# radoslawkrolikowski/financial-market-data-analysis

Hardware: AMD Instinct MI355X
Metric: train seq/sec + 3-class acc, biGRU on synthetic order-book (higher is better)
Workload: dtype bf16; 1 GPU; model=biGRU L2 H128 bidirectional, global_batch=8192, seq_len=120, n_features=96, parallelism=dp1, bench_config=repo

## Files before the change

### fmda_amd/models/bigru.py

```python
from typing import Optional

import numpy as np
import torch
import torch.nn as nn
import torch.nn.functional as F

from ..metrics import batch_metrics


class BiGRU(nn.Module):

    def __init__(self, hidden_size, n_features, output_size, n_layers=1,
                 clip=50, dropout=0.2, spatial_dropout=True,
                 bidirectional=True):
        super().__init__()
        self.hidden_size = hidden_size
        self.n_features = n_features
        self.output_size = output_size
        self.n_layers = n_layers
        self.clip = clip
        self.dropout_p = dropout
        self.spatial_dropout = spatial_dropout
        self.bidirectional = bidirectional
        self.n_directions = 2 if bidirectional else 1
# ... 36 lines not shown
                input_seq = input_seq.permute(0, 2, 1)
                input_seq = self.spatial_dropout1d(input_seq)
                input_seq = input_seq.permute(0, 2, 1)
        elif (self.training and input_seq.is_cuda
              and input_seq.dtype == torch.bfloat16 and self.dropout_p > 0):
            from ..ops.interface import fused_dropout
            input_seq = fused_dropout(input_seq, self.dropout_p)
        else:
            input_seq = self.dropout(input_seq)
        return input_seq

    def _features_after_dropout(self, input_seq: torch.Tensor,
                                hidden: Optional[torch.Tensor] = None
                                ) -> torch.Tensor:
        if input_seq.is_cuda:
            from ..ops.interface import (bigru_stack_raw, pooled_features,
                                         pooled_features_native)
            if pooled_features_native(input_seq, self.hidden_size):
                gru_out, h_last = bigru_stack_raw(
                    input_seq, self.gru, self.n_layers, self.bidirectional,
                    self.dropout_p, self.training, hidden)
                return pooled_features(gru_out, h_last)
            gru_out, h_n = self._gru_hip(input_seq, hidden)
        else:
            gru_out, h_n = self.gru(input_seq, hidden)
        return self._pool_concat(gru_out, h_n)

    def _pool_concat(self, gru_out: torch.Tensor,
                     h_n: torch.Tensor) -> torch.Tensor:
        batch_size = gru_out.size(0)
        input_length = gru_out.size(1)
        hidden_v = h_n.view(self.n_layers, self.n_directions, batch_size,
                            self.hidden_size)
        last_hidden = hidden_v[-1].sum(dim=0)

        if gru_out.is_cuda and self.hidden_size % 2 == 0:
            from ..ops.interface import dirsum_pool
# ... 222 lines not shown
```

### fmda_amd/ops/csrc/bindings.cpp

```cpp
#include <torch/extension.h>
#include <ATen/hip/HIPContext.h>

#include <climits>
#include <cstdint>
#include <vector>

extern "C" int fmda_gru_fwd_launch(int is_bf16, int Hp, const void* gi,
                                   const void* w, const float* bhh, void* out,
                                   float* hlast, int B, int Tseq, int n_dir,
                                   const float* h0, void* out_drop,
                                   unsigned int drop_thr, float drop_scale,
                                   unsigned long long drop_seed,
                                   long gi_pitch, hipStream_t stream);
extern "C" int fmda_gru_fwd_cs_launch(const void* gi, const void* w,
                                      const float* bhh, void* out,
                                      float* hlast, void* hpub,
                                      unsigned int* cnt, int B, int Tseq,
                                      int n_dir, void* out_drop,
                                      unsigned int drop_thr,
                                      float drop_scale,
                                      unsigned long long drop_seed,
                                      long gi_pitch, hipStream_t stream);
extern "C" int fmda_gru_bwd_cs_launch(const void* gi, const void* w,
                                      const void* wt, const float* bhh,
// ... 4 lines not shown
                                      int n_dir, unsigned int drop_thr,
                                      float drop_scale,
                                      unsigned long long drop_seed,
                                      hipStream_t stream);
extern "C" int fmda_gru_bwd_launch(int is_bf16, int Hp, const void* gi,
                                   const void* w, const void* wt,
                                   const float* bhh,
                                   const void* out, const void* dout,
                                   const float* dhT, void* dgi, void* dgh,
                                   float* dh0, float* dbhh, int B, int Tseq,
                                   int n_dir, unsigned int drop_thr,
                                   float drop_scale,
                                   unsigned long long drop_seed,
                                   const float* h0, void* dgh0,
                                   hipStream_t stream);
extern "C" int fmda_mfma_selftest_launch(const void* A, const void* Bm,
                                         float* C, hipStream_t stream);
extern "C" int fmda_pool_fwd_launch(int is_bf16, const void* out, void* maxv,
                                    void* avgv, int* amax, int B, int Tseq,
                                    int H, int n_dir, int act_io, int serial,
                                    hipStream_t stream);
extern "C" int fmda_pool_features_fwd_launch(const void* out,
                                             const float* hlast, void* feat,
                                             int* amax, int B, int Tseq,
                                             int H, int n_dir,
                                             hipStream_t stream);
extern "C" int fmda_pool_features_bwd_launch(const void* dfeat,
                                             const int* amax, void* dout,
                                             float* dhlast, int B, int Tseq,
                                             int H, int n_dir, long ld,
// ... 223 lines not shown
    TORCH_CHECK(T >= 1 && stride >= 1,
                "gru_fwd_windows: T and stride must be >= 1");
    TORCH_CHECK(R >= T, "gru_fwd_windows: table has ", R,
                " rows, fewer than the window T=", T);
    const int64_t nB = (R - T) / stride + 1;
    TORCH_CHECK(nB <= INT_MAX && T <= INT_MAX,
                "gru_fwd_windows: too many windows");
    TORCH_CHECK(reinterpret_cast<uintptr_t>(gi_rows.data_ptr()) % 16 == 0,
                "gru_fwd_windows: gi_rows must be 16-byte aligned");
    return gru_fwd_dispatch(gi_rows, w, bhh, (int)nB, (int)T, n_dir, Hp,
                            is_bf16, stride * row, c10::nullopt, 0.0, 0);
}

std::vector<torch::Tensor> gru_bwd(torch::Tensor gi, torch::Tensor w,
                                   torch::Tensor bhh, torch::Tensor out,
                                   torch::Tensor dout, torch::Tensor dhT,
                                   double drop_p, int64_t drop_seed,
                                   c10::optional<torch::Tensor> h0_opt,
                                   c10::optional<torch::Tensor> wt_opt) {
    int B, T, n_dir, Hp;
    bool is_bf16;
    check_common(gi, w, bhh, B, T, n_dir, Hp, is_bf16);
    const float* h0 = nullptr;
    torch::Tensor dgh0;
    void* dgh0_ptr = nullptr;
    if (h0_opt.has_value()) {
        auto& h = h0_opt.value();
        TORCH_CHECK(h.is_cuda() && h.is_contiguous() &&
                    h.scalar_type() == torch::kFloat32 &&
                    h.sizes() == torch::IntArrayRef({n_dir, B, Hp}),
                    "h0 must be contiguous fp32 (n_dir, B, Hp)");
        h0 = h.data_ptr<float>();
        dgh0 = torch::empty({n_dir, B, (int64_t)3 * Hp}, gi.options());
        dgh0_ptr = dgh0.data_ptr();
    }
    TORCH_CHECK(out.is_contiguous() && dout.is_contiguous() &&
                dhT.is_contiguous(), "fmda gru_bwd: tensors must be contiguous");
    TORCH_CHECK(dhT.scalar_type() == torch::kFloat32, "dhT must be fp32");
    TORCH_CHECK(is_bf16 || Hp <= 256,
                "fp32 backward unsupported for Hp > 256 (LDS budget); "
                "train in bf16 for hidden sizes above 256");
    torch::Tensor dgi, dgh;
    if (getenv("FMDA_ZERO_GRADS")) {
        dgi = torch::zeros_like(gi);
        dgh = torch::zeros_like(gi);
    } else {
        dgi = torch::empty_like(gi);
        dgh = torch::empty_like(gi);
    }
    auto dh0 = torch::empty({n_dir, B, Hp},
                            gi.options().dtype(torch::kFloat32));
    const bool column_split = is_bf16 && Hp == 512 && h0 == nullptr;
    const int64_t db_rows = fmda_gru_bwd_db_rows(is_bf16 ? 1 : 0, Hp, B,
// ... 8 lines not shown
        if (wt_opt.has_value()) {
            wt = wt_opt.value();
            TORCH_CHECK(wt.is_cuda() && wt.is_contiguous() &&
                        wt.scalar_type() == w.scalar_type() &&
                        wt.sizes() == torch::IntArrayRef(
                            {n_dir, Hp, (int64_t)3 * Hp}),
                        "wt must be contiguous (n_dir, Hp, 3Hp) in w's dtype");
        } else {
            wt = w.transpose(1, 2).contiguous();
        }
        wt_ptr = wt.data_ptr();
    }
    auto stream = at::hip::getCurrentHIPStream();
    int rc;
    const DropParams dp = drop_params(drop_p);
    if (column_split) {
        const unsigned int cs_thr = dp.thr;
        const float cs_scale = dp.scale;
        const int BR = 256;
        const int GB = (B + BR - 1) / BR;
        const int G = GB * n_dir;
        auto gpub = torch::empty({2, G, BR, (int64_t)3 * Hp}, gi.options());
        auto cnt = torch::zeros({G}, gi.options().dtype(torch::kUInt32));
        rc = fmda_gru_bwd_cs_launch(
            gi.data_ptr(), w.data_ptr(), wt_ptr, bhh.data_ptr<float>(),
            out.data_ptr(), dout.data_ptr(), dhT.data_ptr<float>(),
            dgi.data_ptr(), dgh.data_ptr(), dh0.data_ptr<float>(),
            dbpart.data_ptr<float>(), gpub.data_ptr(),
            (unsigned int*)cnt.data_ptr(), B, T, n_dir, cs_thr, cs_scale,
            (unsigned long long)drop_seed, stream.stream());
    } else {
// ... 606 lines not shown
          "table (shared rows, no materialised windows)",
          py::arg("gi_rows"), py::arg("w"), py::arg("bhh"), py::arg("T"),
          py::arg("stride") = 1);
    m.def("normalize_table", &normalize_table,
          "nan_to_num + min/max normalisation of a raw (N, F) table",
          py::arg("x"), py::arg("x_min"), py::arg("x_max"), py::arg("dtype"));
    m.def("window_batch", &window_batch,
          "gather windows of a table into a (B, T, F) batch with fused "
          "(spatial) input dropout",
          py::arg("table"), py::arg("starts"), py::arg("window"),
          py::arg("p"), py::arg("seed"), py::arg("spatial"));
    m.def("gru_bwd", &gru_bwd, "fused biGRU recurrence backward (HIP/CDNA4)",
          py::arg("gi"), py::arg("w"), py::arg("bhh"), py::arg("out"),
          py::arg("dout"), py::arg("dhT"), py::arg("drop_p") = 0.0,
          py::arg("drop_seed") = 0, py::arg("h0") = py::none(),
          py::arg("wt") = py::none());
    m.def("mfma_selftest", &mfma_selftest, "mfma fragment layout self-test");
    m.def("dropout_fused", &dropout_fused,
          "counter-based dropout (mask recomputed in backward)");
    m.def("spatial_dropout_fused", &spatial_dropout_fused,
          "channel (Dropout2d) dropout over (B, T, F) without permutes");
    m.def("ingest_row", &ingest_row,
          "streaming ingest: shift GPU window ring + normalize new row");
    m.def("pool_concat_infer", &pool_concat_infer,
          "fused [dirsum(h_last) | max | avg] concat for inference");
    m.def("head_sigmoid", &head_sigmoid,
          "linear head + sigmoid emitting probabilities");
    m.def("pool_fwd", &pool_fwd, "fused dirsum+max/avg pooling forward",
          py::arg("out"), py::arg("n_dir"), py::arg("act_dtype") = false,
          py::arg("serial") = false);
    m.def("pool_features_fwd", &pool_features_fwd,
// ... 40 lines not shown
```

### fmda_amd/ops/csrc/gru_kernels.hip

```cpp
#include <hip/hip_runtime.h>
#include <hip/hip_bf16.h>

#include "dropout_common.h"

#define FMDA_DEV __device__ __forceinline__

typedef __bf16 bf16x8_t __attribute__((ext_vector_type(8)));
typedef float f32x4_t __attribute__((ext_vector_type(4)));

namespace fmda {

#define FMDA_LOG2E 1.4426950408889634f

FMDA_DEV float fast_exp2(float x) { return __builtin_amdgcn_exp2f(x); }
FMDA_DEV float fast_rcp(float x) { return __builtin_amdgcn_rcpf(x); }

FMDA_DEV float sigmoidf(float x) {
    return fast_rcp(1.0f + fast_exp2(-x * FMDA_LOG2E));
}

FMDA_DEV float fast_tanh(float x) {
    return 1.0f - 2.0f * fast_rcp(1.0f + fast_exp2(2.0f * FMDA_LOG2E * x));
}

// ... 1074 lines not shown
                ((__bf16*)out_b)[(long)tt * out_trow + j] = hb;
            }
        }
        asm volatile("s_waitcnt lgkmcnt(0)" ::: "memory");
        __builtin_amdgcn_s_barrier();
    }

    if ((lane >> 4) == 0) {
        float* hl = hlast + (long)dir * Hp;
#pragma unroll
        for (int i = 0; i < CPW; ++i)
            hl[(wave + NW * i) * 16 + lane] = hreg[i];
    }
}

template <int BT, int Hp, int NT, int WPE, int PHASES = 7>
__global__ __attribute__((amdgpu_flat_work_group_size(NT, NT),
                          amdgpu_waves_per_eu(WPE, WPE)))
void gru_bwd_v3_kernel(const __hip_bfloat16* __restrict__ gi,
                       const __hip_bfloat16* __restrict__ w,
                       const __hip_bfloat16* __restrict__ wt,
                       const float* __restrict__ bhh,
                       const __hip_bfloat16* __restrict__ out,
                       const __hip_bfloat16* __restrict__ dout,
                       const float* __restrict__ dhT,
                       __hip_bfloat16* __restrict__ dgi,
                       __hip_bfloat16* __restrict__ dgh, float* __restrict__ dh0,
                       float* __restrict__ dbhh, int B, int Tseq, int n_dir,
                       unsigned int drop_thr, float drop_scale,
                       unsigned long long drop_seed,
                       const float* __restrict__ h0,
                       __hip_bfloat16* __restrict__ dgh0) {
    constexpr int NW = NT / 64;
    constexpr int MT = BT / 16;
    constexpr int NCT = Hp / 16;
    constexpr int CPW = NCT / NW;
    constexpr int KK = Hp / 32;
    constexpr int KK2 = (3 * Hp) / 32;
    constexpr int GP = 3 * Hp;
    constexpr int HROW = Hp * 2;
    constexpr int GP3 = 3 * Hp + 8;
    constexpr int PW = (BT * GP * 2) / 1024 / NW;
    constexpr int DOP = (BT * HROW) / 1024 / NW;
    constexpr int HBP = DOP;
    constexpr int NST = 2 * ((BT * GP * 2) / 16) / NT;
    static_assert(NCT % NW == 0 && (BT * GP * 2) % (1024 * NW) == 0 &&
                  (BT * HROW) % (1024 * NW) == 0, "tiling mismatch");
// ... 1 lines not shown
    const int tid = threadIdx.x;
    const int wave = tid >> 6;
    const int lane = tid & 63;
    const int b0 = blockIdx.x * BT;
    const int dir = blockIdx.y;
    const bool rev = (dir == 1);
    const int rows_valid = min(BT, B - b0);

    extern __shared__ __attribute__((aligned(16))) char smem[];
    char* p = smem;
    __hip_bfloat16* gi_s0 = (__hip_bfloat16*)p; p += 2 * BT * GP;
    __hip_bfloat16* gi_s1 = (__hip_bfloat16*)p; p += 2 * BT * GP;
    __hip_bfloat16* gi_s2 = (__hip_bfloat16*)p; p += 2 * BT * GP;
    __hip_bfloat16* hb_s0 = (__hip_bfloat16*)p; p += BT * HROW;
    __hip_bfloat16* hb_s1 = (__hip_bfloat16*)p; p += BT * HROW;
    __hip_bfloat16* do_s0 = (__hip_bfloat16*)p; p += BT * HROW;
    __hip_bfloat16* do_s1 = (__hip_bfloat16*)p; p += BT * HROW;
    __hip_bfloat16* dgh_s0 = (__hip_bfloat16*)p; p += 2 * BT * GP3;
    __hip_bfloat16* dgh_s1 = (__hip_bfloat16*)p; p += 2 * BT * GP3;
    float* bhh_s = (float*)p;
    auto dgh_buf = [&](int b) { return b ? dgh_s1 : dgh_s0; };
    auto gi_slot = [&](int sl) {
        return sl == 0 ? gi_s0 : (sl == 1 ? gi_s1 : gi_s2);
    };
    auto hb_buf = [&](int b) { return b ? hb_s1 : hb_s0; };
    auto do_buf = [&](int b) { return b ? do_s1 : do_s0; };

    const long gi_row = (long)Tseq * n_dir * 3 * Hp;
    const long out_row = (long)Tseq * n_dir * Hp;
    const __hip_bfloat16* gi_b = gi + (long)b0 * gi_row + (long)dir * 3 * Hp;
    __hip_bfloat16* dgi_b = dgi + (long)b0 * gi_row + (long)dir * 3 * Hp;
    __hip_bfloat16* dgh_b = dgh + (long)b0 * gi_row + (long)dir * 3 * Hp;
    const __hip_bfloat16* out_b = out + (long)b0 * out_row + (long)dir * Hp;
    const __hip_bfloat16* dout_b = dout + (long)b0 * out_row + (long)dir * Hp;

    for (int c = tid; c < 3 * Hp; c += NT)
        bhh_s[c] = bhh[(long)dir * 3 * Hp + c];

    const __hip_bfloat16* wdir = w + (long)dir * 3 * Hp * Hp;
    const __hip_bfloat16* wt_dir = wt + (long)dir * Hp * 3 * Hp;
    bf16x8_t wA[CPW][3][KK];
    bf16x8_t wB[CPW][KK2];
#pragma unroll
    for (int i = 0; i < CPW; ++i) {
        const int ct = wave + NW * i;
        const int jcol = ct * 16 + (lane & 15);
        const __bf16* wtrow = (const __bf16*)wt_dir + (long)jcol * 3 * Hp;
#pragma unroll
        for (int g = 0; g < 3; ++g)
#pragma unroll
            for (int kk = 0; kk < KK; ++kk)
                wA[i][g][kk] = load_wfragA<Hp>(wdir, Hp, ct, g, kk, lane);
#pragma unroll
// ... 3 lines not shown

    float dhreg[CPW][MT][4];
    float dbacc[CPW][4];
#pragma unroll
    for (int i = 0; i < CPW; ++i) {
#pragma unroll
        for (int g = 0; g < 4; ++g) dbacc[i][g] = 0.0f;
        const int ct = wave + NW * i;
        const int j = ct * 16 + (lane & 15);
        const float* hT = dhT + ((long)dir * B + b0) * Hp;
#pragma unroll
        for (int m = 0; m < MT; ++m)
#pragma unroll
            for (int e = 0; e < 4; ++e) {
                const int b = 16 * m + 4 * (lane >> 4) + e;
                dhreg[i][m][e] =
                    (b < rows_valid) ? hT[(long)b * Hp + j] : 0.0f;
            }
    }

    const int wavu = __builtin_amdgcn_readfirstlane(wave);
    auto glds_gi = [&](int tt, int sl) {
        const __hip_bfloat16* src_t = gi_b + (long)tt * n_dir * 3 * Hp;
        __hip_bfloat16* dst = gi_slot(sl);
#pragma unroll
        for (int k = 0; k < PW; ++k) {
            const int off = (wavu * PW + k) * 1024 + lane * 16;
            const int e = off >> 1;
            int r = e / GP;
            const int c = e % GP;
            if (r >= rows_valid) r = 0;
            glds16(src_t + (long)r * gi_row + c,
// ... 43 lines not shown
        for (int c = tid; c < BT * Hp; c += NT)
            ((__bf16*)hb_buf(buf))[c] = (__bf16)0.0f;
    };
    auto hb_read = [&](const __hip_bfloat16* hb, int b, int j) -> float {
        const int k16 = (j * 2) >> 4;
        const int ksw = k16 ^ (b & 15);
        const int within = (j * 2) & 15;
        return (float)*(const __bf16*)((const char*)hb + b * HROW +
                                       ksw * 16 + within);
    };

    {
        const int u = Tseq - 1;
        const int tt = rev ? 0 : u;
        glds_gi(tt, u % 3);
        glds_do(tt, u & 1);
        if (u > 0) {
            const int ttp = rev ? 1 : (u - 1);
            glds_hb(ttp, u & 1);
        } else {
            zero_hb(u & 1);
        }
        asm volatile("s_waitcnt vmcnt(0)" ::: "memory");
        asm volatile("s_waitcnt lgkmcnt(0)" ::: "memory");
        __builtin_amdgcn_s_barrier();
    }

    for (int u = Tseq - 1; u >= 0; --u) {
        const int q = u & 1;
        const int slot = u % 3;
        const int tt = rev ? (Tseq - 1 - u) : u;
        const bool have_next = (u > 0);
        const bool have_prev = (u + 1 < Tseq);

        if (have_next) {
            const int ttn = rev ? (Tseq - u) : (u - 1);
            glds_gi(ttn, (u - 1) % 3);
            glds_do(ttn, 1 - q);
            if (u >= 2)
                glds_hb(rev ? (Tseq + 1 - u) : (u - 2), 1 - q);
            else
                zero_hb(1 - q);
        }
        if (have_prev) {
            const int ttp = rev ? (Tseq - 2 - u) : (u + 1);
            store_tile<__hip_bfloat16, BT, NT>(
                gi_slot((u + 1) % 3), dgi_b + (long)ttp * n_dir * 3 * Hp, GP, GP,
                gi_row, rows_valid, tid);
            const int sh = rev ? (ttp + 1) : (ttp - 1);
            store_tile<__hip_bfloat16, BT, NT>(
                dgh_buf(1 - q), dgh_b + (long)sh * n_dir * 3 * Hp, GP, GP3,
                gi_row, rows_valid, tid);
        }
// ... 24 lines not shown
#pragma unroll
                    for (int m = 0; m < MT; ++m)
                        acc[i][g][m] = __builtin_amdgcn_mfma_f32_16x16x32_bf16(
                            a[m], wA[i][g][kk], acc[i][g][m], 0, 0, 0);
            }
        }
#pragma unroll
        for (int i = 0; PHASES & 2 && i < CPW; ++i) {
            const int ct = wave + NW * i;
            const int j = ct * 16 + (lane & 15);
            __bf16* grow = (__bf16*)gi_slot(slot);
            __bf16* dgrow = (__bf16*)dgh_buf(q);
            const __bf16* dorow = (const __bf16*)do_buf(q);
#pragma unroll
            for (int m = 0; m < MT; ++m) {
#pragma unroll
                for (int e = 0; e < 4; ++e) {
                    const int b = 16 * m + 4 * (lane >> 4) + e;
                    const bool live = (b < rows_valid);
                    const float gr = acc[i][0][m][e] + bhh_s[j];
                    const float gz = acc[i][1][m][e] + bhh_s[Hp + j];
                    const float hn = acc[i][2][m][e] + bhh_s[2 * Hp + j];
                    const float ir = (float)grow[b * GP + j];
                    const float iz = (float)grow[b * GP + Hp + j];
                    const float in_ = (float)grow[b * GP + 2 * Hp + j];
                    const float r = sigmoidf(ir + gr);
                    const float z = sigmoidf(iz + gz);
                    const float n = fast_tanh(in_ + r * hn);
                    const float hprev = hb_read(hbq, b, j);
                    float doval = live ? (float)dorow[b * Hp + j] : 0.0f;
                    if (drop_thr != 0u) {
                        const long o = ((long)(b0 + b) * Tseq + tt) *
                                           n_dir * Hp +
                                       (long)dir * Hp + j;
                        const unsigned long long rnd =
                            mix64(drop_seed ^ (unsigned long long)(o >> 3));
                        const unsigned int u =
                            (unsigned int)(rnd >> (8 * ((int)o & 7))) & 0xFF;
                        doval = (u < drop_thr) ? 0.0f : doval * drop_scale;
                    }
                    const float dht = dhreg[i][m][e] + doval;
                    const float dz_pre =
                        live ? dht * (hprev - n) * z * (1.0f - z) : 0.0f;
                    const float dn_pre =
                        live ? dht * (1.0f - z) * (1.0f - n * n) : 0.0f;
                    const float dr_pre =
// ... 1680 lines not shown
                               hipStream_t stream) {
    constexpr int Hp = 128;
    const size_t lds = 3 * 2 * BT * 3 * Hp + 2 * 2 * BT * Hp +
                       2 * 2 * BT * Hp + 2 * 2 * BT * (3 * Hp + 8) +
                       4 * 3 * Hp;
    auto k = gru_bwd_v3_kernel<BT, Hp, NT, 2, PHASES>;
    (void)hipFuncSetAttribute((const void*)k,
        hipFuncAttributeMaxDynamicSharedMemorySize, (int)lds);
    const dim3 grid((B + BT - 1) / BT, n_dir);
    k<<<grid, NT, lds, stream>>>(
        (const __hip_bfloat16*)gi, (const __hip_bfloat16*)w,
        (const __hip_bfloat16*)wt, bhh,
        (const __hip_bfloat16*)out, (const __hip_bfloat16*)dout, dhT,
        (__hip_bfloat16*)dgi, (__hip_bfloat16*)dgh, dh0, dbhh, B, Tseq,
        n_dir, drop_thr, drop_scale, drop_seed, h0,
        (__hip_bfloat16*)dgh0);
    return 0;
}

static bool bwd_v3_bt16() {
    static const bool small = getenv("FMDA_BWD_BT16") != nullptr;
    return small;
}

static int launch_bwd_v3_128(const void* gi, const void* w, const void* wt,
                             const float* bhh,
                             const void* out, const void* dout,
                             const float* dhT, void* dgi, void* dgh,
                             float* dh0, float* dbhh, int B, int Tseq,
                             int n_dir, unsigned int drop_thr,
                             float drop_scale, unsigned long long drop_seed,
// ... 205 lines not shown
        }
    } else {
        switch (Hp) {
            case 16: G(float, 32, 16, false, 256, false); break;
            case 32: G(float, 32, 32, false, 256, false); break;
            case 64: G(float, 32, 64, false, 256, false); break;
            case 128: G(float, 32, 128, false, 256, false); break;
            case 256: G(float, 16, 256, false, 256, false); break;
            default: return -1;
        }
    }
#undef G
    return hipGetLastError() == hipSuccess ? 0 : -4;
}

extern "C" int fmda_mfma_selftest_launch(const void* A, const void* Bm,
                                         float* C, hipStream_t stream) {
    mfma_selftest_kernel<<<1, 64, 0, stream>>>((const __hip_bfloat16*)A,
                                               (const __hip_bfloat16*)Bm, C);
    return hipGetLastError() == hipSuccess ? 0 : 1;
}

}
```

### fmda_amd/ops/interface.py

```python
import os
from typing import List, Optional, Tuple

import torch

from . import load_extension
from .blas import (chunked_colsum, chunked_outer, chunked_outer_parts,
                   enable_tunableop, split_chunks)

_ALLOWED_HP = [32, 64, 128, 256, 512]


def _pad_h(H: int) -> int:
    for hp in _ALLOWED_HP:
        if H <= hp:
            return hp
    raise ValueError(f"hidden size {H} > {_ALLOWED_HP[-1]} not supported")


def _glue_mode() -> int:
    return {"0": 0, "2": 2}.get(os.environ.get("FMDA_NATIVE_GLUE", "1"), 1)


def _native_glue() -> bool:
    return _glue_mode() >= 1
# ... 231 lines not shown
                   for g in (dmax, davg)):
                dmax, davg = dmax.contiguous(), davg.contiguous()
        else:
            dmax, davg = dmax.float().contiguous(), davg.float().contiguous()
        dout = ext.pool_bwd(dmax, davg, amax, T, n_dir, dtype)
        return dout, None


def dirsum_pool(out: torch.Tensor, n_dir: int):
    return _DirSumPool.apply(out, n_dir)


class _PooledFeatures(torch.autograd.Function):

    @staticmethod
    def forward(ctx, out, h_last):
        ext = load_extension()
        feat, amax = ext.pool_features_fwd(out.contiguous(),
                                           h_last.contiguous())
        ctx.save_for_backward(amax)
        ctx.meta = (out.shape[1], h_last.shape[0])
        return feat

    @staticmethod
    def backward(ctx, dfeat):
        ext = load_extension()
        (amax,) = ctx.saved_tensors
        T, n_dir = ctx.meta
        if (dfeat.dtype != torch.bfloat16 or dfeat.stride(1) != 1
                or dfeat.stride(0) < dfeat.shape[1]):
            dfeat = dfeat.to(torch.bfloat16).contiguous()
        d_out, d_hlast = ext.pool_features_bwd(dfeat, amax, T, n_dir)
        return d_out, d_hlast


_POOL_SMALL_GRID = 4096


def pooled_features_native(x: torch.Tensor, H: int) -> bool:
    return (_native_glue() and x.is_cuda and x.dtype == torch.bfloat16
            and H % 8 == 0 and H <= _ALLOWED_HP[-1] and _pad_h(H) == H
            and x.shape[0] * (H // 2) >= _POOL_SMALL_GRID)


def pooled_features(out: torch.Tensor, h_last: torch.Tensor) -> torch.Tensor:
    return _PooledFeatures.apply(out, h_last)


# ... 74 lines not shown
    return _HeadLoss.apply(x2d, Wc, bc, y.float(), wgt.float(), pw.float())


def _unpad_gate_rows(w, H, Hp):
    if H == Hp:
        return w
    return torch.cat([w[g * Hp:g * Hp + H] for g in range(3)], dim=0)


class _BiGRULayer(torch.autograd.Function):

    @staticmethod
    def forward(ctx, x, Hp, w_ih0, w_hh0, b_ih0, b_hh0,
                w_ih1, w_hh1, b_ih1, b_hh1, out_drop_p=0.0,
                out_drop_seed=0, h0=None):
        ext = load_extension()
        D = 2 if w_ih1 is not None else 1
        H = w_hh0.shape[1]
        dtype = x.dtype
        B, T, F = x.shape
        params = [(w_ih0, w_hh0, b_ih0, b_hh0)]
        if D == 2:
            params.append((w_ih1, w_hh1, b_ih1, b_hh1))
        with torch.no_grad():
            w_ih_cat, b_ih_cat, w_hh_cat, b_hh_cat, wt = _pack_layer(
                params, H, Hp, dtype)
        x2d = x.reshape(B * T, F)
        gi = torch.addmm(b_ih_cat, x2d, w_ih_cat.t()).view(B, T, -1)
        h0c = h0.detach().contiguous() if h0 is not None else None
        res = ext.gru_fwd(gi, w_hh_cat, b_hh_cat, h0c, out_drop_p,
                          out_drop_seed)
        out, h_last = res[0], res[1]
        ctx.save_for_backward(x2d, w_ih_cat, w_hh_cat, b_hh_cat, gi, out, wt)
        ctx.h0 = h0c
        ctx.meta = (D, H, Hp, out_drop_p, out_drop_seed)
        ctx.native_reductions = _native_reductions()
        ctx.native_glue = _native_glue()
        ctx.set_materialize_grads(False)
        if len(res) > 2:
            return out, h_last, res[2]
        return out, h_last

    @staticmethod
    def backward(ctx, d_out, d_hlast, d_outdrop=None):
        ext = load_extension()
        x2d, w_ih_cat, w_hh_cat, b_hh_cat, gi, out, wt = ctx.saved_tensors
        D, H, Hp, drop_p, drop_seed = ctx.meta
        need_dx = ctx.needs_input_grad[0]
        if drop_p > 0:
            assert d_out is None, "unexpected grad on raw out with fused dropout"
            d_out = d_outdrop
        if d_out is None:
            d_out = torch.zeros_like(out)
        if d_hlast is None:
            d_hlast = out.new_zeros(
                (w_hh_cat.shape[0], out.shape[0], Hp), dtype=torch.float32)
        d_out = d_out.contiguous().to(gi.dtype)
        d_hlast = d_hlast.contiguous().float()
        h0c = ctx.h0
        res = ext.gru_bwd(gi, w_hh_cat, b_hh_cat, out, d_out, d_hlast,
                          drop_p, drop_seed, h0c, wt)
        dgi, dgh, dh0_out, dbhh, dbih = res[:5]
        dgh0 = res[5] if len(res) > 5 else None
        M = dgi.shape[0] * dgi.shape[1]
        dx = None
        if need_dx:
            dx = torch.matmul(dgi.reshape(M, -1), w_ih_cat)
            dx = dx.view(dgi.shape[0], dgi.shape[1], -1)
        dh0_grad = dh0_out if h0c is not None else None

        if wt is not None and ctx.native_reductions and dgh0 is None:
            wg = ext.finalize_gru_wgrads(
                chunked_outer_parts(dgi.reshape(M, -1), x2d),
                chunked_outer_parts(dgh.reshape(M, -1), out.reshape(M, -1)),
                D, H, Hp)
            wgrads = [(wg[2 * d], wg[2 * d + 1]) for d in range(D)]
# ... 20 lines not shown
                dwhh = cross[d * 3 * Hp:(d + 1) * 3 * Hp,
                             d * Hp:(d + 1) * Hp].contiguous()
                wgrads.append((_unpad_gate_rows(dwih, H, Hp),
                               _unpad_gate_rows(dwhh, H, Hp)[:, :H]))

        grads = [wgrads[d] + (_unpad_gate_rows(dbih[d], H, Hp),
                              _unpad_gate_rows(dbhh[d], H, Hp))
                 for d in range(D)]
        if D == 1:
            grads.append((None, None, None, None))
        (a0, b0, c0, e0), (a1, b1, c1, e1) = grads
        return (dx, None, a0, b0, c0, e0, a1, b1, c1, e1, None, None,
                dh0_grad)



_PACK_EPOCH = 0


def _packed_inference_weights(gru_module, layer, params, Hp, H, dtype):
    key = f"_fmda_pack_l{layer}_{dtype}_{params[0][0].device}"
    flat = [t for four in params for t in four]
    versions = (_PACK_EPOCH,) + tuple(t._version for t in flat)
    ent = getattr(gru_module, key, None)
    if ent is not None and ent[0] == versions:
        return ent[1]
    packed = _pack_layer(params, H, Hp, dtype)[:4]
    setattr(gru_module, key, (versions, packed))
    return packed

# ... 32 lines not shown
                ) -> Tuple[torch.Tensor, torch.Tensor]:
    out, h_n, _ = _bigru_stack(x, gru_module, n_layers, bidirectional,
                               dropout_p, training, hidden)
    return out, h_n


def bigru_stack_raw(x: torch.Tensor, gru_module: torch.nn.GRU, n_layers: int,
                    bidirectional: bool, dropout_p: float, training: bool,
                    hidden: Optional[torch.Tensor] = None
                    ) -> Tuple[torch.Tensor, torch.Tensor]:
    out, _, h_last = _bigru_stack(x, gru_module, n_layers, bidirectional,
                                  dropout_p, training, hidden, need_h_n=False)
    return out, h_last


def _bigru_stack(x, gru_module, n_layers, bidirectional, dropout_p, training,
                 hidden=None, need_h_n=True):
    enable_tunableop()
    D = 2 if bidirectional else 1
    H = gru_module.hidden_size
    Hp = _pad_h(H)

    h0_layers = [None] * n_layers
    if hidden is not None:
        B = x.shape[0]
        assert hidden.shape == (n_layers * D, B, H), \
            f"hidden must be ({n_layers * D}, {B}, {H})"
        hid32 = hidden.float()
        for layer in range(n_layers):
            h0_layers[layer] = _pad_cols(
                hid32[layer * D:(layer + 1) * D], H, Hp).contiguous()

    h_n_parts: List[torch.Tensor] = []
    inp = x
    for layer in range(n_layers):
        p = _layer_params(gru_module, layer, D)
        drop_here = (training and dropout_p > 0 and layer < n_layers - 1)
        defer = (drop_here and Hp == H and Hp in (128, 512)
                 and x.dtype == torch.bfloat16 and x.is_cuda
                 and (Hp == 128 or (h0_layers[layer] is None
                      and os.environ.get("FMDA_CS_DROP", "1") != "0")))
        seed = (int(torch.empty((), dtype=torch.int64).random_())
                if defer else 0)
        dp = (dropout_p, seed) if defer else (0.0, 0)

        h0_l = h0_layers[layer]
        dropped_pad = None
        if not training and not torch.is_grad_enabled():
            out_pad, h_last = _infer_layer(gru_module, layer, p, Hp, H, inp,
                                           h0_l)
        elif D == 2:
            res = _BiGRULayer.apply(inp, Hp, *p[0], *p[1], *dp, h0_l)
            out_pad, h_last = res[0], res[1]
            dropped_pad = res[2] if len(res) > 2 else None
        else:
            res = _BiGRULayer.apply(inp, Hp, *p[0],
                                    None, None, None, None, *dp, h0_l)
            out_pad, h_last = res[0], res[1]
            dropped_pad = res[2] if len(res) > 2 else None

        out = _unpad_out(out_pad, H, Hp, D)
        if need_h_n:
            h_n_parts.append(h_last[:, :, :H].to(x.dtype))

        inp = out
        if drop_here:
            if defer:
                inp = dropped_pad
            else:
                inp = fused_dropout(inp, dropout_p)

    h_n = torch.cat(h_n_parts, dim=0) if need_h_n else None
    return inp, h_n, h_last


def table_projections(table: torch.Tensor, gru_module: torch.nn.GRU,
                      bidirectional: bool) -> torch.Tensor:
    assert not torch.is_grad_enabled(), "windowed inference runs under no_grad"
    enable_tunableop()
    D = 2 if bidirectional else 1
    H = gru_module.hidden_size
    Hp = _pad_h(H)
    w_ih_cat, b_ih_cat, _, _ = _packed_inference_weights(
        gru_module, 0, _layer_params(gru_module, 0, D), Hp, H, table.dtype)
    return torch.addmm(b_ih_cat, table, w_ih_cat.t())

# ... 29 lines not shown
```

Before: 1.100 million seq/s.

## Fuse pooled-feature backward into top-layer GRU backward kernel

```diff
diff --git a/fmda_amd/models/bigru.py b/fmda_amd/models/bigru.py
--- a/fmda_amd/models/bigru.py
+++ b/fmda_amd/models/bigru.py
@@ -74,13 +74,12 @@
                                 hidden: Optional[torch.Tensor] = None
                                 ) -> torch.Tensor:
         if input_seq.is_cuda:
-            from ..ops.interface import (bigru_stack_raw, pooled_features,
+            from ..ops.interface import (bigru_stack_features,
                                          pooled_features_native)
             if pooled_features_native(input_seq, self.hidden_size):
-                gru_out, h_last = bigru_stack_raw(
+                return bigru_stack_features(
                     input_seq, self.gru, self.n_layers, self.bidirectional,
                     self.dropout_p, self.training, hidden)
-                return pooled_features(gru_out, h_last)
             gru_out, h_n = self._gru_hip(input_seq, hidden)
         else:
             gru_out, h_n = self.gru(input_seq, hidden)
diff --git a/fmda_amd/ops/csrc/bindings.cpp b/fmda_amd/ops/csrc/bindings.cpp
--- a/fmda_amd/ops/csrc/bindings.cpp
+++ b/fmda_amd/ops/csrc/bindings.cpp
@@ -42,6 +42,15 @@
                                    unsigned long long drop_seed,
                                    const float* h0, void* dgh0,
                                    hipStream_t stream);
+extern "C" int fmda_gru_bwd_pooled_available();
+extern "C" int fmda_gru_bwd_pooled_launch(const void* gi, const void* w,
+                                          const void* wt, const float* bhh,
+                                          const void* out, const void* dfeat,
+                                          const int* amax, long ld, void* dgi,
+                                          void* dgh, float* dh0, float* dbhh,
+                                          int B, int Tseq, int n_dir,
+                                          const float* h0, void* dgh0,
+                                          hipStream_t stream);
 extern "C" int fmda_mfma_selftest_launch(const void* A, const void* Bm,
                                          float* C, hipStream_t stream);
 extern "C" int fmda_pool_fwd_launch(int is_bf16, const void* out, void* maxv,
@@ -295,13 +304,61 @@
 
 std::vector<torch::Tensor> gru_bwd(torch::Tensor gi, torch::Tensor w,
                                    torch::Tensor bhh, torch::Tensor out,
-                                   torch::Tensor dout, torch::Tensor dhT,
+                                   c10::optional<torch::Tensor> dout_opt,
+                                   c10::optional<torch::Tensor> dhT_opt,
                                    double drop_p, int64_t drop_seed,
                                    c10::optional<torch::Tensor> h0_opt,
-                                   c10::optional<torch::Tensor> wt_opt) {
+                                   c10::optional<torch::Tensor> wt_opt,
+                                   c10::optional<torch::Tensor> dfeat_opt,
+                                   c10::optional<torch::Tensor> amax_opt) {
     int B, T, n_dir, Hp;
     bool is_bf16;
     check_common(gi, w, bhh, B, T, n_dir, Hp, is_bf16);
+    const bool pooled = dfeat_opt.has_value() || amax_opt.has_value();
+    torch::Tensor dout, dhT, dfeat, amax;
+    long dfeat_ld = 0;
+    if (pooled) {
+        TORCH_CHECK(dfeat_opt.has_value() && amax_opt.has_value() &&
+                    !dout_opt.has_value() && !dhT_opt.has_value(),
+                    "fmda gru_bwd: pass either (dout, dhT) or (dfeat, amax)");
+        dfeat = dfeat_opt.value();
+        amax = amax_opt.value();
+        TORCH_CHECK(is_bf16 && Hp == 128,
+                    "fmda gru_bwd: the pooled path needs bf16 and "
+                    "H == Hp == 128, got Hp=", Hp);
+        TORCH_CHECK(T <= 256, "fmda gru_bwd: the pooled path keeps amax in "
+                    "one byte, T=", T, " > 256");
+        TORCH_CHECK(drop_p == 0.0,
+                    "fmda gru_bwd: the pooled path has no dropout");
+        TORCH_CHECK(fmda_gru_bwd_pooled_available() == 1,
+                    "fmda gru_bwd: no pooled variant of the kernel selected "
+                    "by FMDA_BWD_BT16 / FMDA_BWD_PHASES");
+        TORCH_CHECK(dfeat.is_cuda() && dfeat.dim() == 2 &&
+                    dfeat.scalar_type() == torch::kBFloat16 &&
+                    dfeat.size(0) == B && dfeat.size(1) == 3 * Hp,
+                    "fmda gru_bwd: dfeat must be bf16 (B, 3H) on the GPU");
+        TORCH_CHECK(amax.is_cuda() && amax.is_contiguous() &&
+                    amax.scalar_type() == torch::kInt32 && amax.dim() == 2 &&
+                    amax.size(0) == B && amax.size(1) == Hp,
+                    "fmda gru_bwd: amax must be contiguous int32 (B, H)");
+        TORCH_CHECK(dfeat.stride(1) == 1,
+                    "fmda gru_bwd: dfeat needs unit column stride");
+        dfeat_ld = B == 1 ? 3L * Hp : (long)dfeat.stride(0);
+        TORCH_CHECK(dfeat_ld >= 3 * Hp && dfeat_ld % 8 == 0 &&
+                    reinterpret_cast<uintptr_t>(dfeat.data_ptr()) % 16 == 0 &&
+                    reinterpret_cast<uintptr_t>(amax.data_ptr()) % 16 == 0,
+                    "fmda gru_bwd: dfeat needs a row pitch >= 3H that is a "
+                    "multiple of 8 and 16-byte aligned data");
+        TORCH_CHECK(out.is_cuda() && out.scalar_type() == gi.scalar_type() &&
+                    out.dim() == 3 && out.size(0) == B && out.size(1) == T &&
+                    out.size(2) == (int64_t)n_dir * Hp,
+                    "fmda gru_bwd: out must be (B, T, n_dir*Hp)");
+    } else {
+        TORCH_CHECK(dout_opt.has_value() && dhT_opt.has_value(),
+                    "fmda gru_bwd: dout and dhT are required");
+        dout = dout_opt.value();
+        dhT = dhT_opt.value();
+    }
     const float* h0 = nullptr;
     torch::Tensor dgh0;
     void* dgh0_ptr = nullptr;
@@ -315,9 +372,11 @@
         dgh0 = torch::empty({n_dir, B, (int64_t)3 * Hp}, gi.options());
         dgh0_ptr = dgh0.data_ptr();
     }
-    TORCH_CHECK(out.is_contiguous() && dout.is_contiguous() &&
-                dhT.is_contiguous(), "fmda gru_bwd: tensors must be contiguous");
-    TORCH_CHECK(dhT.scalar_type() == torch::kFloat32, "dhT must be fp32");
+    TORCH_CHECK(out.is_contiguous() &&
+                (pooled || (dout.is_contiguous() && dhT.is_contiguous())),
+                "fmda gru_bwd: tensors must be contiguous");
+    TORCH_CHECK(pooled || dhT.scalar_type() == torch::kFloat32,
+                "dhT must be fp32");
     TORCH_CHECK(is_bf16 || Hp <= 256,
                 "fp32 backward unsupported for Hp > 256 (LDS budget); "
                 "train in bf16 for hidden sizes above 256");
@@ -356,7 +415,15 @@
     auto stream = at::hip::getCurrentHIPStream();
     int rc;
     const DropParams dp = drop_params(drop_p);
-    if (column_split) {
+    if (pooled) {
+        TORCH_CHECK(wt_ptr != nullptr, "fmda gru_bwd: pooled path needs wt");
+        rc = fmda_gru_bwd_pooled_launch(
+            gi.data_ptr(), w.data_ptr(), wt_ptr, bhh.data_ptr<float>(),
+            out.data_ptr(), dfeat.data_ptr(), amax.data_ptr<int>(), dfeat_ld,
+            dgi.data_ptr(), dgh.data_ptr(), dh0.data_ptr<float>(),
+            dbpart.data_ptr<float>(), B, T, n_dir, h0, dgh0_ptr,
+            stream.stream());
+    } else if (column_split) {
         const unsigned int cs_thr = dp.thr;
         const float cs_scale = dp.scale;
         const int BR = 256;
@@ -993,7 +1060,11 @@
           py::arg("gi"), py::arg("w"), py::arg("bhh"), py::arg("out"),
           py::arg("dout"), py::arg("dhT"), py::arg("drop_p") = 0.0,
           py::arg("drop_seed") = 0, py::arg("h0") = py::none(),
-          py::arg("wt") = py::none());
+          py::arg("wt") = py::none(), py::arg("dfeat") = py::none(),
+          py::arg("amax") = py::none());
+    m.def("gru_bwd_pooled_available",
+          []() { return fmda_gru_bwd_pooled_available() == 1; },
+          "whether gru_bwd(dfeat=, amax=) has a kernel in this process");
     m.def("mfma_selftest", &mfma_selftest, "mfma fragment layout self-test");
     m.def("dropout_fused", &dropout_fused,
           "counter-based dropout (mask recomputed in backward)");
diff --git a/fmda_amd/ops/csrc/gru_kernels.hip b/fmda_amd/ops/csrc/gru_kernels.hip
--- a/fmda_amd/ops/csrc/gru_kernels.hip
+++ b/fmda_amd/ops/csrc/gru_kernels.hip
@@ -1112,7 +1112,8 @@
     }
 }
 
-template <int BT, int Hp, int NT, int WPE, int PHASES = 7>
+template <int BT, int Hp, int NT, int WPE, int PHASES = 7,
+          bool POOLED = false>
 __global__ __attribute__((amdgpu_flat_work_group_size(NT, NT),
                           amdgpu_waves_per_eu(WPE, WPE)))
 void gru_bwd_v3_kernel(const __hip_bfloat16* __restrict__ gi,
@@ -1128,7 +1129,9 @@
                        unsigned int drop_thr, float drop_scale,
                        unsigned long long drop_seed,
                        const float* __restrict__ h0,
-                       __hip_bfloat16* __restrict__ dgh0) {
+                       __hip_bfloat16* __restrict__ dgh0,
+                       const __hip_bfloat16* __restrict__ dfeat,
+                       const int* __restrict__ amax, long dfeat_ld) {
     constexpr int NW = NT / 64;
     constexpr int MT = BT / 16;
     constexpr int NCT = Hp / 16;
@@ -1160,8 +1163,11 @@
     __hip_bfloat16* gi_s2 = (__hip_bfloat16*)p; p += 2 * BT * GP;
     __hip_bfloat16* hb_s0 = (__hip_bfloat16*)p; p += BT * HROW;
     __hip_bfloat16* hb_s1 = (__hip_bfloat16*)p; p += BT * HROW;
-    __hip_bfloat16* do_s0 = (__hip_bfloat16*)p; p += BT * HROW;
+    __hip_bfloat16* do_s0 = (__hip_bfloat16*)p;
+    unsigned int* pv_s = (unsigned int*)p; p += BT * HROW;
     __hip_bfloat16* do_s1 = (__hip_bfloat16*)p; p += BT * HROW;
+    unsigned int* im_s = (unsigned int*)p;
+    if (POOLED) p += BT * Hp;
     __hip_bfloat16* dgh_s0 = (__hip_bfloat16*)p; p += 2 * BT * GP3;
     __hip_bfloat16* dgh_s1 = (__hip_bfloat16*)p; p += 2 * BT * GP3;
     float* bhh_s = (float*)p;
@@ -1183,6 +1189,56 @@
     for (int c = tid; c < 3 * Hp; c += NT)
         bhh_s[c] = bhh[(long)dir * 3 * Hp + c];
 
+    if (POOLED) {
+        constexpr int H8 = Hp / 8;
+        unsigned short* gl_s = (unsigned short*)dgh_s0;
+        for (int c = tid; c < BT * H8; c += NT) {
+            const int b = c / H8;
+            const int h8 = (c % H8) * 8;
+            bf16x8_t dl, dm, da;
+            int4 a0 = make_int4(0, 0, 0, 0), a1 = a0;
+            const bool rowlive = (b < rows_valid);
+            if (rowlive) {
+                const __hip_bfloat16* dr =
+                    dfeat + (long)(b0 + b) * dfeat_ld + h8;
+                dl = *(const bf16x8_t*)dr;
+                dm = *(const bf16x8_t*)(dr + Hp);
+                da = *(const bf16x8_t*)(dr + 2 * Hp);
+                const int* ai = amax + (long)(b0 + b) * Hp + h8;
+                a0 = *(const int4*)ai;
+                a1 = *(const int4*)(ai + 4);
+            }
+            const int imv[8] = {a0.x, a0.y, a0.z, a0.w,
+                                a1.x, a1.y, a1.z, a1.w};
+            const int ct = h8 >> 4;
+            const int im0 = (ct / NW) * MT + (b >> 4);
+            const int e = b & 3;
+            const int t0 = (ct % NW) * 64 + 16 * ((b >> 2) & 3) + (h8 & 15);
+#pragma unroll
+            for (int k = 0; k < 8; ++k) {
+                unsigned int pv = 0u, iv = 0u;
+                unsigned short gl = 0;
+                if (rowlive) {
+                    const float ga = (float)da[k] / (float)Tseq;
+                    const float gm = (float)dm[k];
+                    const __bf16 v0 = (__bf16)__float2bfloat16(ga + 0.0f);
+                    const __bf16 v1 = (__bf16)__float2bfloat16(ga + gm);
+                    pv = (unsigned int)__builtin_bit_cast(unsigned short, v0) |
+                         ((unsigned int)__builtin_bit_cast(unsigned short, v1)
+                          << 16);
+                    iv = (unsigned int)imv[k];
+                    gl = __builtin_bit_cast(unsigned short, (__bf16)dl[k]);
+                }
+                pv_s[(im0 * 4 + e) * NT + t0 + k] = pv;
+                ((unsigned char*)im_s)[(im0 * NT + t0 + k) * 4 + e] =
+                    (unsigned char)iv;
+                gl_s[(im0 * 4 + e) * NT + t0 + k] = gl;
+            }
+        }
+        asm volatile("s_waitcnt lgkmcnt(0)" ::: "memory");
+        __builtin_amdgcn_s_barrier();
+    }
+
     const __hip_bfloat16* wdir = w + (long)dir * 3 * Hp * Hp;
     const __hip_bfloat16* wt_dir = wt + (long)dir * Hp * 3 * Hp;
     bf16x8_t wA[CPW][3][KK];
@@ -1216,8 +1272,14 @@
 #pragma unroll
             for (int e = 0; e < 4; ++e) {
                 const int b = 16 * m + 4 * (lane >> 4) + e;
-                dhreg[i][m][e] =
-                    (b < rows_valid) ? hT[(long)b * Hp + j] : 0.0f;
+                if (POOLED) {
+                    const unsigned short gl = ((const unsigned short*)
+                        dgh_s0)[((i * MT + m) * 4 + e) * NT + tid];
+                    dhreg[i][m][e] = __uint_as_float((unsigned int)gl << 16);
+                } else {
+                    dhreg[i][m][e] =
+                        (b < rows_valid) ? hT[(long)b * Hp + j] : 0.0f;
+                }
             }
     }
 
@@ -1291,7 +1353,7 @@
         const int u = Tseq - 1;
         const int tt = rev ? 0 : u;
         glds_gi(tt, u % 3);
-        glds_do(tt, u & 1);
+        if (!POOLED) glds_do(tt, u & 1);
         if (u > 0) {
             const int ttp = rev ? 1 : (u - 1);
             glds_hb(ttp, u & 1);
@@ -1313,7 +1375,7 @@
         if (have_next) {
             const int ttn = rev ? (Tseq - u) : (u - 1);
             glds_gi(ttn, (u - 1) % 3);
-            glds_do(ttn, 1 - q);
+            if (!POOLED) glds_do(ttn, 1 - q);
             if (u >= 2)
                 glds_hb(rev ? (Tseq + 1 - u) : (u - 2), 1 - q);
             else
@@ -1368,6 +1430,8 @@
             const __bf16* dorow = (const __bf16*)do_buf(q);
 #pragma unroll
             for (int m = 0; m < MT; ++m) {
+                unsigned int imw = 0u;
+                if (POOLED) imw = im_s[(i * MT + m) * NT + tid];
 #pragma unroll
                 for (int e = 0; e < 4; ++e) {
                     const int b = 16 * m + 4 * (lane >> 4) + e;
@@ -1382,8 +1446,18 @@
                     const float z = sigmoidf(iz + gz);
                     const float n = fast_tanh(in_ + r * hn);
                     const float hprev = hb_read(hbq, b, j);
-                    float doval = live ? (float)dorow[b * Hp + j] : 0.0f;
-                    if (drop_thr != 0u) {
+                    float doval;
+                    if (POOLED) {
+                        const unsigned int pv =
+                            pv_s[((i * MT + m) * 4 + e) * NT + tid];
+                        const int im = (int)((imw >> (8 * e)) & 0xFFu);
+                        const unsigned int bits =
+                            (tt == im) ? (pv & 0xFFFF0000u) : (pv << 16);
+                        doval = live ? __uint_as_float(bits) : 0.0f;
+                    } else {
+                        doval = live ? (float)dorow[b * Hp + j] : 0.0f;
+                    }
+                    if (!POOLED && drop_thr != 0u) {
                         const long o = ((long)(b0 + b) * Tseq + tt) *
                                            n_dir * Hp +
                                        (long)dir * Hp + j;
@@ -3094,7 +3168,36 @@
         (const __hip_bfloat16*)out, (const __hip_bfloat16*)dout, dhT,
         (__hip_bfloat16*)dgi, (__hip_bfloat16*)dgh, dh0, dbhh, B, Tseq,
         n_dir, drop_thr, drop_scale, drop_seed, h0,
-        (__hip_bfloat16*)dgh0);
+        (__hip_bfloat16*)dgh0, nullptr, nullptr, 0L);
+    return 0;
+}
+
+static int launch_bwd_v3_128_pooled(const void* gi, const void* w,
+                                    const void* wt, const float* bhh,
+                                    const void* out, const void* dfeat,
+                                    const int* amax, long ld, void* dgi,
+                                    void* dgh, float* dh0, float* dbhh,
+                                    int B, int Tseq, int n_dir,
+                                    const float* h0, void* dgh0,
+                                    hipStream_t stream) {
+    constexpr int Hp = 128, BT = 32, NT = 512;
+    const size_t lds = 3 * 2 * BT * 3 * Hp + 2 * 2 * BT * Hp +
+                       (4 * BT * Hp + BT * Hp) + 2 * 2 * BT * (3 * Hp + 8) +
+                       4 * 3 * Hp;
+    static_assert(3 * 2 * BT * 3 * Hp + 2 * 2 * BT * Hp + 5 * BT * Hp +
+                  2 * 2 * BT * (3 * Hp + 8) + 4 * 3 * Hp <= 160 * 1024,
+                  "pooled table does not fit the LDS");
+    auto k = gru_bwd_v3_kernel<BT, Hp, NT, 2, 7, true>;
+    (void)hipFuncSetAttribute((const void*)k,
+        hipFuncAttributeMaxDynamicSharedMemorySize, (int)lds);
+    const dim3 grid((B + BT - 1) / BT, n_dir);
+    k<<<grid, NT, lds, stream>>>(
+        (const __hip_bfloat16*)gi, (const __hip_bfloat16*)w,
+        (const __hip_bfloat16*)wt, bhh,
+        (const __hip_bfloat16*)out, nullptr, nullptr,
+        (__hip_bfloat16*)dgi, (__hip_bfloat16*)dgh, dh0, dbhh, B, Tseq,
+        n_dir, 0u, 1.0f, 0ull, h0, (__hip_bfloat16*)dgh0,
+        (const __hip_bfloat16*)dfeat, amax, ld);
     return 0;
 }
 
@@ -3330,6 +3433,26 @@
     return hipGetLastError() == hipSuccess ? 0 : -4;
 }
 
+extern "C" int fmda_gru_bwd_pooled_available() {
+    static const bool phases = getenv("FMDA_BWD_PHASES") != nullptr;
+    return (bwd_v3_bt16() || phases) ? 0 : 1;
+}
+
+extern "C" int fmda_gru_bwd_pooled_launch(const void* gi, const void* w,
+                                          const void* wt, const float* bhh,
+                                          const void* out, const void* dfeat,
+                                          const int* amax, long ld, void* dgi,
+                                          void* dgh, float* dh0, float* dbhh,
+                                          int B, int Tseq, int n_dir,
+                                          const float* h0, void* dgh0,
+                                          hipStream_t stream) {
+    if (!fmda_gru_bwd_pooled_available()) return -8;
+    if (Tseq < 1 || Tseq > 256 || ld < 3 * 128 || ld % 8 != 0) return -9;
+    launch_bwd_v3_128_pooled(gi, w, wt, bhh, out, dfeat, amax, ld, dgi, dgh,
+                             dh0, dbhh, B, Tseq, n_dir, h0, dgh0, stream);
+    return hipGetLastError() == hipSuccess ? 0 : -4;
+}
+
 extern "C" int fmda_mfma_selftest_launch(const void* A, const void* Bm,
                                          float* C, hipStream_t stream) {
     mfma_selftest_kernel<<<1, 64, 0, stream>>>((const __hip_bfloat16*)A,
diff --git a/fmda_amd/ops/interface.py b/fmda_amd/ops/interface.py
--- a/fmda_amd/ops/interface.py
+++ b/fmda_amd/ops/interface.py
@@ -269,24 +269,36 @@
 class _PooledFeatures(torch.autograd.Function):
 
     @staticmethod
-    def forward(ctx, out, h_last):
-        ext = load_extension()
+    def forward(ctx, out, h_last, *layer):
+        ext = load_extension()
+        saved = ()
+        ctx.fused = bool(layer)
+        if layer:
+            (out, h_last), saved = _BiGRULayer.run_forward(
+                ctx, *layer[:10], 0.0, 0, layer[10])
         feat, amax = ext.pool_features_fwd(out.contiguous(),
                                            h_last.contiguous())
-        ctx.save_for_backward(amax)
-        ctx.meta = (out.shape[1], h_last.shape[0])
+        ctx.save_for_backward(*saved, amax)
+        ctx.pool_meta = (out.shape[1], h_last.shape[0])
         return feat
 
     @staticmethod
     def backward(ctx, dfeat):
         ext = load_extension()
-        (amax,) = ctx.saved_tensors
-        T, n_dir = ctx.meta
+        *saved, amax = ctx.saved_tensors
+        T, n_dir = ctx.pool_meta
         if (dfeat.dtype != torch.bfloat16 or dfeat.stride(1) != 1
-                or dfeat.stride(0) < dfeat.shape[1]):
+                or dfeat.stride(0) < dfeat.shape[1]
+                or (ctx.fused and dfeat.stride(0) % 8 != 0)):
             dfeat = dfeat.to(torch.bfloat16).contiguous()
-        d_out, d_hlast = ext.pool_features_bwd(dfeat, amax, T, n_dir)
-        return d_out, d_hlast
+        if not ctx.fused:
+            d_out, d_hlast = ext.pool_features_bwd(dfeat, amax, T, n_dir)
+            return d_out, d_hlast
+        if dfeat.data_ptr() % 16 != 0:
+            dfeat = dfeat.clone(memory_format=torch.contiguous_format)
+        g = _BiGRULayer.run_backward(ctx, tuple(saved), None, None,
+                                     dfeat=dfeat, amax=amax, x_index=2)
+        return (None, None) + g[:10] + (g[12],)
 
 
 _POOL_SMALL_GRID = 4096
@@ -391,6 +403,16 @@
     def forward(ctx, x, Hp, w_ih0, w_hh0, b_ih0, b_hh0,
                 w_ih1, w_hh1, b_ih1, b_hh1, out_drop_p=0.0,
                 out_drop_seed=0, h0=None):
+        res, saved = _BiGRULayer.run_forward(
+            ctx, x, Hp, w_ih0, w_hh0, b_ih0, b_hh0, w_ih1, w_hh1, b_ih1,
+            b_hh1, out_drop_p, out_drop_seed, h0)
+        ctx.save_for_backward(*saved)
+        return res
+
+    @staticmethod
+    def run_forward(ctx, x, Hp, w_ih0, w_hh0, b_ih0, b_hh0,
+                    w_ih1, w_hh1, b_ih1, b_hh1, out_drop_p, out_drop_seed,
+                    h0):
         ext = load_extension()
         D = 2 if w_ih1 is not None else 1
         H = w_hh0.shape[1]
@@ -408,22 +430,32 @@
         res = ext.gru_fwd(gi, w_hh_cat, b_hh_cat, h0c, out_drop_p,
                           out_drop_seed)
         out, h_last = res[0], res[1]
-        ctx.save_for_backward(x2d, w_ih_cat, w_hh_cat, b_hh_cat, gi, out, wt)
+        saved = (x2d, w_ih_cat, w_hh_cat, b_hh_cat, gi, out, wt)
         ctx.h0 = h0c
         ctx.meta = (D, H, Hp, out_drop_p, out_drop_seed)
         ctx.native_reductions = _native_reductions()
         ctx.native_glue = _native_glue()
         ctx.set_materialize_grads(False)
         if len(res) > 2:
-            return out, h_last, res[2]
-        return out, h_last
+            return (out, h_last, res[2]), saved
+        return (out, h_last), saved
 
     @staticmethod
     def backward(ctx, d_out, d_hlast, d_outdrop=None):
-        ext = load_extension()
-        x2d, w_ih_cat, w_hh_cat, b_hh_cat, gi, out, wt = ctx.saved_tensors
+        return _BiGRULayer.run_backward(ctx, ctx.saved_tensors, d_out,
+                                        d_hlast, d_outdrop)
+
+    @staticmethod
+    def run_backward(ctx, saved, d_out, d_hlast, d_outdrop=None,
+                     dfeat=None, amax=None, x_index=0):
+        ext = load_extension()
+        x2d, w_ih_cat, w_hh_cat, b_hh_cat, gi, out, wt = saved
         D, H, Hp, drop_p, drop_seed = ctx.meta
-        need_dx = ctx.needs_input_grad[0]
+        need_dx = ctx.needs_input_grad[x_index]
+        if dfeat is not None:
+            res = ext.gru_bwd(gi, w_hh_cat, b_hh_cat, out, None, None,
+                              0.0, 0, ctx.h0, wt, dfeat, amax)
+            return _BiGRULayer.finish_backward(ctx, saved, res, need_dx)
         if drop_p > 0:
             assert d_out is None, "unexpected grad on raw out with fused dropout"
             d_out = d_outdrop
@@ -437,6 +469,14 @@
         h0c = ctx.h0
         res = ext.gru_bwd(gi, w_hh_cat, b_hh_cat, out, d_out, d_hlast,
                           drop_p, drop_seed, h0c, wt)
+        return _BiGRULayer.finish_backward(ctx, saved, res, need_dx)
+
+    @staticmethod
+    def finish_backward(ctx, saved, res, need_dx):
+        ext = load_extension()
+        x2d, w_ih_cat, w_hh_cat, b_hh_cat, gi, out, wt = saved
+        D, H, Hp, _, _ = ctx.meta
+        h0c = ctx.h0
         dgi, dgh, dh0_out, dbhh, dbih = res[:5]
         dgh0 = res[5] if len(res) > 5 else None
         M = dgi.shape[0] * dgi.shape[1]
@@ -487,6 +527,16 @@
                 dh0_grad)
 
 
+def _fused_pool_bwd() -> bool:
+    return os.environ.get("FMDA_FUSED_POOL_BWD", "1") != "0"
+
+
+def fused_pool_bwd_native(x: torch.Tensor, H: int) -> bool:
+    return (_fused_pool_bwd() and pooled_features_native(x, H)
+            and H == 128 and x.shape[1] <= 256 and torch.is_grad_enabled()
+            and load_extension().gru_bwd_pooled_available())
+
+
 
 _PACK_EPOCH = 0
 
@@ -549,12 +599,25 @@
     return out, h_last
 
 
+def bigru_stack_features(x: torch.Tensor, gru_module: torch.nn.GRU,
+                         n_layers: int, bidirectional: bool,
+                         dropout_p: float, training: bool,
+                         hidden: Optional[torch.Tensor] = None
+                         ) -> torch.Tensor:
+    feat, _, _ = _bigru_stack(x, gru_module, n_layers, bidirectional,
+                              dropout_p, training, hidden, need_h_n=False,
+                              pooled=True)
+    return feat
+
+
 def _bigru_stack(x, gru_module, n_layers, bidirectional, dropout_p, training,
-                 hidden=None, need_h_n=True):
+                 hidden=None, need_h_n=True, pooled=False):
     enable_tunableop()
     D = 2 if bidirectional else 1
     H = gru_module.hidden_size
     Hp = _pad_h(H)
+    assert not (pooled and need_h_n)
+    fuse_top = pooled and fused_pool_bwd_native(x, H)
 
     h0_layers = [None] * n_layers
     if hidden is not None:
@@ -584,6 +647,10 @@
         if not training and not torch.is_grad_enabled():
             out_pad, h_last = _infer_layer(gru_module, layer, p, Hp, H, inp,
                                            h0_l)
+        elif fuse_top and training and layer == n_layers - 1:
+            p1 = p[1] if D == 2 else (None, None, None, None)
+            return (_PooledFeatures.apply(None, None, inp, Hp, *p[0], *p1,
+                                          h0_l), None, None)
         elif D == 2:
             res = _BiGRULayer.apply(inp, Hp, *p[0], *p[1], *dp, h0_l)
             out_pad, h_last = res[0], res[1]
@@ -605,6 +672,8 @@
             else:
                 inp = fused_dropout(inp, dropout_p)
 
+    if pooled:
+        return pooled_features(inp, h_last), None, None
     h_n = torch.cat(h_n_parts, dim=0) if need_h_n else None
     return inp, h_n, h_last
 
```

New measurement: 1.143 million seq/s, median of 6. 3.9% higher.
